# cule/multimot_track

Hardware: AMD Instinct MI355X
Metric: KITTI RGB-D frames/sec (ego+object poses) at 1/2/4/8 GPUs; CPU ref fps (higher is better)
Workload: dtype u8

## Files before the change

### multimot_track_amd/csrc/mmt_ba.hip

```cpp

#include <hip/hip_runtime.h>

#include <algorithm>
#include <cfloat>
#include <chrono>
#include <cstdio>
#include <climits>
#include <cmath>
#include <cstring>
#include <map>

#include "mmt_ba.h"
#include "mmt_devmath.h"
#include "mmt_internal.h"

namespace mmt {

namespace {

constexpr int kBAThreads = 512;
constexpr int kBAWaves = kBAThreads / 64;
constexpr int kLdsRows = 96;

struct BAWork {
// ... 126 lines not shown
  Jp[0][0] = x * y / z_2 * c.fx;
  Jp[0][1] = -(1 + (x * x / z_2)) * c.fx;
  Jp[0][2] = y / z * c.fx;
  Jp[0][3] = -1. / z * c.fx;
  Jp[0][4] = 0;
  Jp[0][5] = x / z_2 * c.fx;
  Jp[1][0] = (1 + y * y / z_2) * c.fy;
  Jp[1][1] = -x * y / z_2 * c.fy;
  Jp[1][2] = -x / z * c.fy;
  Jp[1][3] = 0;
  Jp[1][4] = -1. / z * c.fy;
  Jp[1][5] = y / z_2 * c.fy;
  if (stereo) {
    Jp[2][0] = Jp[0][0] - c.bf * y / z_2;
    Jp[2][1] = Jp[0][1] + c.bf * x / z_2;
    Jp[2][2] = Jp[0][2];
    Jp[2][3] = Jp[0][3];
    Jp[2][4] = 0;
    Jp[2][5] = Jp[0][5] - c.bf / z_2;
  } else {
#pragma unroll
    for (int k = 0; k < 6; k++) Jp[2][k] = 0;
  }
}

__device__ __forceinline__ void inverse3(const double (&m)[9], double (&r)[9]) {
#define COF(i, j)                                                                           \
  (m[3 * (((i) + 1) % 3) + ((j) + 1) % 3] * m[3 * (((i) + 2) % 3) + ((j) + 2) % 3] -         \
   m[3 * (((i) + 1) % 3) + ((j) + 2) % 3] * m[3 * (((i) + 2) % 3) + ((j) + 1) % 3])
  const double c0 = COF(0, 0), c1 = COF(1, 0), c2 = COF(2, 0);
  const double det = c0 * m[0] + c1 * m[3] + c2 * m[6];
  const double invdet = 1.0 / det;
  r[0] = c0 * invdet;
  r[1] = c1 * invdet;
  r[2] = c2 * invdet;
  r[3] = COF(0, 1) * invdet;
  r[4] = COF(1, 1) * invdet;
  r[5] = COF(2, 1) * invdet;
  r[6] = COF(0, 2) * invdet;
  r[7] = COF(1, 2) * invdet;
  r[8] = COF(2, 2) * invdet;
#undef COF
}

__device__ __forceinline__ double wg_sum1(double v, double* part) {
  v = wave_sum_dpp(v);
  const int lane = threadIdx.x & 63, wave = threadIdx.x >> 6;
  if (lane == 0) part[wave] = v;
  __syncthreads();
  double s = 0;
#pragma unroll
  for (int w = 0; w < kBAWaves; w++) s += part[w];
  __syncthreads();
  return s;
}

__device__ __forceinline__ double wg_max1(double v, double* part) {
#pragma unroll
  for (int o = 32; o > 0; o >>= 1) v = fmax(v, __shfl_xor(v, o, 64));
  const int lane = threadIdx.x & 63, wave = threadIdx.x >> 6;
  if (lane == 0) part[wave] = v;
  __syncthreads();
  double m = 0;
#pragma unroll
  for (int w = 0; w < kBAWaves; w++) m = fmax(m, part[w]);
  __syncthreads();
  return m;
}

__device__ __forceinline__ void wave_sync_lds() {
  __builtin_amdgcn_fence(__ATOMIC_RELEASE, "wavefront");
  __builtin_amdgcn_wave_barrier();
  __builtin_amdgcn_fence(__ATOMIC_ACQUIRE, "wavefront");
}

}

namespace {

constexpr int kMkThreads = 256;
constexpr int kMkWaves = kMkThreads / 64;
constexpr int kMkSolveThreads = 512;
constexpr int kMkDecideThreads = 1024;

struct BAState {
  int done, round, iter, qmax, need_lin, lam_init, cb, ok2, nBad, nact;
  int spec_ok;
  int it_done[2], trials[2];
  double lambda, ni, chk, currentChi, iniChi, scale_p;
  long long prof[8];
};

struct BAWork2 {
  BAState* st;
  DSE3* pose;
  double* X;
  double* Hll;
  double* bl;
  double* Dinv;
  double* err;
  double* Hpl;
  double* Hpe;
  double* Y;
  double* cv;
  double* Hpp;
  double* bp;
  double* cvs;
  double* Sblk;
  double* x;
  double* S;
  double* vec;
  const int4* kitem;
  const int* kitem_start;
  const int4* bitem;
  const int* bitem_start;
  int n_kitem, n_bitem;
  double* Hpart;
  double* Spart;
  double* cvpart;
  double* linpart;
  double* p4part;
  unsigned* p4cnt;
  uint8_t* level;
  int* eopt;
  uint8_t* kf_act;
  uint8_t* pt_act;
  int gP;
  int gPp;
  const int* heavy;
  int n_heavy;
  double* hres;
  int spec;
};

template <int K, int NW>
__device__ __forceinline__ void wg_sumK(const double (&v)[K], double* part, double* out) {
  const int lane = threadIdx.x & 63, wave = threadIdx.x >> 6;
  double mine = 0;
#pragma unroll
  for (int q = 0; q < K; q++) {
    const double s = wave_sum_dpp(v[q]);
    if (lane == q) mine = s;
  }
  if (lane < K) part[wave * K + lane] = mine;
  __syncthreads();
  if ((int)threadIdx.x < K) {
    double s = 0;
#pragma unroll
    for (int w = 0; w < NW; w++) s += part[w * K + threadIdx.x];
    out[threadIdx.x] = s;
  }
  __syncthreads();
}

template <int NW>
__device__ __forceinline__ double wg_maxN(double v, double* part) {
#pragma unroll
  for (int o = 32; o > 0; o >>= 1) v = fmax(v, __shfl_xor(v, o, 64));
  const int lane = threadIdx.x & 63, wave = threadIdx.x >> 6;
  if (lane == 0) part[wave] = v;
  __syncthreads();
  double m = 0;
#pragma unroll
  for (int w = 0; w < NW; w++) m = fmax(m, part[w]);
  __syncthreads();
  return m;
}

__device__ __forceinline__ int ba2_diag_q(int r) { return 6 * r - r * (r - 1) / 2; }

template <int U = 8>
__device__ __forceinline__ double ordered_sum(const double* base, size_t stride, int b, int e) {
  double s = 0;
  for (int it = b; it < e; it += U) {
    double v[U];
#pragma unroll
    for (int u = 0; u < U; u++) v[u] = base[stride * (size_t)min(it + u, e - 1)];
#pragma unroll
    for (int u = 0; u < U; u++)
      if (it + u < e) s += v[u];
  }
  return s;
}

__device__ __forceinline__ double ba2_hsum(const BAWork2& w, int a, int q) {
  return ordered_sum(w.Hpart + q, 27, w.kitem_start[a], w.kitem_start[a + 1]);
}

__device__ __forceinline__ double ba2_lambda_init(const BADesc& d, const BAWork2& w, double* sh) {
  if (threadIdx.x < 64) {
    double m = 0;
    for (int g = threadIdx.x; g < w.gP; g += 64) m = fmax(m, w.linpart[2 * g + 1]);
    for (int q = threadIdx.x; q < 6 * d.n_opt; q += 64) {
      const int a = q / 6;
      if (w.kf_act[d.opt_kf[a]]) m = fmax(m, fabs(ba2_hsum(w, a, ba2_diag_q(q % 6))));
    }
#pragma unroll
    for (int o = 32; o > 0; o >>= 1) m = fmax(m, __shfl_xor(m, o, 64));
    if (threadIdx.x == 0) *sh = 1e-5 * m;
  }
  __syncthreads();
  return *sh;
}

__device__ __forceinline__ Cam ba_cam(const BADesc& d) { return Cam{d.fx, d.fy, d.cx, d.cy, d.bf}; }

__device__ __forceinline__ double huber_mono() { return (double)(float)sqrt(5.991); }
__device__ __forceinline__ double huber_stereo() { return (double)(float)sqrt(7.815); }

__global__ __launch_bounds__(kMkThreads) void k_ba2_init(BADesc d, BAWork2 w) {
  const int gt = blockIdx.x * kMkThreads + threadIdx.x, gs = gridDim.x * kMkThreads;
  const size_t n6 = 6 * (size_t)d.n_opt;
  for (int j = gt; j < d.n_pt; j += gs) {
    for (int r = 0; r < 3; r++) {
// ... 113 lines not shown
  return r0;
}

template <int K>
__device__ __forceinline__ void ba2_wave_ordered_add(double* sh, int lane, int n, const bool valid,
                                                     const double (&v)[K], double (&sum)[K]) {
#pragma unroll
  for (int q = 0; q < K; q++) sh[K * lane + q] = valid ? v[q] : 0.0;
  const unsigned long long vb = __ballot(valid);
  __builtin_amdgcn_fence(__ATOMIC_RELEASE, "wavefront");
  __builtin_amdgcn_wave_barrier();
  __builtin_amdgcn_fence(__ATOMIC_ACQUIRE, "wavefront");
  for (int k = 0; k < n; k++) {
    if (!((vb >> k) & 1ull)) continue;
#pragma unroll
    for (int q = 0; q < K; q++) sum[q] += sh[K * k + q];
  }
  __builtin_amdgcn_fence(__ATOMIC_RELEASE, "wavefront");
  __builtin_amdgcn_wave_barrier();
}

__device__ __forceinline__ double ba2_lin_point(const BADesc& d, const BAWork2& w, int j,
                                               const DSE3* pose, const double (&X)[3], bool robust,
                                               int lb, double* mx) {
  double* Hpl_b = w.Hpl + (size_t)lb * 18 * d.n_edge;
  double* Hpe_b = w.Hpe + (size_t)lb * 27 * d.n_edge;
  double chi = 0;
  {
    double hl[9] = {0, 0, 0, 0, 0, 0, 0, 0, 0}, b3[3] = {0, 0, 0};
    for (int e = d.pt_start[j]; e < d.pt_start[j + 1]; e++) {
      if (w.level[e]) continue;
      double acc9[9], g3[3];
      chi += ba2_lin_edge(d, w, e, pose, X, robust, Hpl_b, Hpe_b, acc9, g3);
#pragma unroll
      for (int q = 0; q < 9; q++) hl[q] += acc9[q];
#pragma unroll
      for (int a = 0; a < 3; a++) b3[a] += g3[a];
    }
    double* Hll_b = w.Hll + (size_t)lb * 9 * d.n_pt;
    double* bl_b = w.bl + (size_t)lb * 3 * d.n_pt;
#pragma unroll
    for (int q = 0; q < 9; q++) Hll_b[9 * (size_t)j + q] = hl[q];
#pragma unroll
    for (int q = 0; q < 3; q++) bl_b[3 * (size_t)j + q] = b3[q];
    *mx = fmax(fabs(hl[0]), fmax(fabs(hl[4]), fabs(hl[8])));
  }
  return chi;
}

__device__ __forceinline__ double ba2_lin_point_wave(const BADesc& d, const BAWork2& w, int j,
                                                    const DSE3* pose, const double (&X)[3],
                                                    bool robust, int lb, double* mx, double* sh) {
  const int lane = threadIdx.x & 63;
  double* Hpl_b = w.Hpl + (size_t)lb * 18 * d.n_edge;
  double* Hpe_b = w.Hpe + (size_t)lb * 27 * d.n_edge;
  double sum[13] = {0, 0, 0, 0, 0, 0, 0, 0, 0, 0, 0, 0, 0};
  const int e1 = d.pt_start[j + 1];
  for (int e0 = d.pt_start[j]; e0 < e1; e0 += 64) {
    const int e = e0 + lane;
    const bool valid = e < e1 && !w.level[e];
    double v[13];
    if (valid) {
      double acc9[9], g3[3];
      v[0] = ba2_lin_edge(d, w, e, pose, X, robust, Hpl_b, Hpe_b, acc9, g3);
#pragma unroll
      for (int q = 0; q < 9; q++) v[1 + q] = acc9[q];
#pragma unroll
      for (int q = 0; q < 3; q++) v[10 + q] = g3[q];
    }
    ba2_wave_ordered_add<13>(sh, lane, min(64, e1 - e0), valid, v, sum);
  }
  if (lane == 0) {
    double* Hll_b = w.Hll + (size_t)lb * 9 * d.n_pt;
    double* bl_b = w.bl + (size_t)lb * 3 * d.n_pt;
#pragma unroll
    for (int q = 0; q < 9; q++) Hll_b[9 * (size_t)j + q] = sum[1 + q];
#pragma unroll
    for (int q = 0; q < 3; q++) bl_b[3 * (size_t)j + q] = sum[10 + q];
  }
  *mx = fmax(fabs(sum[1]), fmax(fabs(sum[5]), fabs(sum[9])));
  return sum[0];
}

__global__ __launch_bounds__(kMkThreads) void k_ba2_lin(BADesc d, BAWork2 w) {
  __shared__ double s_part[2 * kMkWaves];
  const BAState* st = w.st;
  if (st->done || !st->need_lin || st->spec_ok) return;
  const bool robust = st->round == 0;
  const int cb = st->cb;
  const DSE3* pose = w.pose + (size_t)cb * d.n_kf;
  const double* Xc = w.X + (size_t)cb * 3 * d.n_pt;
  const int j = blockIdx.x * kMkThreads + threadIdx.x;
  double chi = 0, mx = 0;
  if (j < d.n_pt) {
    double m = 0;
    if (ba2_heavy(d, j)) {
      chi = w.hres[2 * (size_t)j];
      m = w.hres[2 * (size_t)j + 1];
    } else {
      const double X[3] = {Xc[3 * (size_t)j], Xc[3 * (size_t)j + 1], Xc[3 * (size_t)j + 2]};
      chi = ba2_lin_point(d, w, j, pose, X, robust, cb, &m);
    }
    if (w.pt_act[j]) mx = m;
  }
  const double cs = wave_sum_dpp(chi);
  const int lane = threadIdx.x & 63, wave = threadIdx.x >> 6;
  if (lane == 0) s_part[wave] = cs;
  const double m = wg_maxN<kMkWaves>(mx, s_part + kMkWaves);
  if (threadIdx.x == 0) {
    double t = 0;
#pragma unroll
    for (int q = 0; q < kMkWaves; q++) t += s_part[q];
    w.linpart[2 * blockIdx.x] = t;
    w.linpart[2 * blockIdx.x + 1] = m;
  }
}

__global__ __launch_bounds__(kMkThreads) void k_ba2_lin_heavy(BADesc d, BAWork2 w) {
  __shared__ double s_stage[kMkWaves][64 * 13];
  const BAState* st = w.st;
  if (st->done || !st->need_lin || st->spec_ok) return;
  const int wave = threadIdx.x >> 6;
  const int hi = (int)blockIdx.x * kMkWaves + wave;
  if (hi >= w.n_heavy) return;
  const int cb = st->cb;
  const DSE3* pose = w.pose + (size_t)cb * d.n_kf;
  const double* Xc = w.X + (size_t)cb * 3 * d.n_pt;
  const int j = w.heavy[hi];
  const double X[3] = {Xc[3 * (size_t)j], Xc[3 * (size_t)j + 1], Xc[3 * (size_t)j + 2]};
  double m = 0;
  const double c = ba2_lin_point_wave(d, w, j, pose, X, st->round == 0, cb, &m, s_stage[wave]);
  if ((threadIdx.x & 63) == 0) {
    w.hres[2 * (size_t)j] = c;
    w.hres[2 * (size_t)j + 1] = m;
  }
}

__global__ __launch_bounds__(kMkThreads) void k_ba2_kfsum(BADesc d, BAWork2 w) {
  __shared__ double s_part[27 * kMkWaves];
  __shared__ double s_out[32];
  const BAState* st = w.st;
  if (st->done || !st->need_lin) return;
  const int4 it = w.kitem[blockIdx.x];
  const int t = it.y + threadIdx.x;
  double acc[27];
#pragma unroll
  for (int q = 0; q < 27; q++) acc[q] = 0;
  if (t < it.z) {
    const int e = d.kf_edges[t];
    if (!w.level[e]) {
      const double* h = &w.Hpe[(size_t)st->cb * 27 * d.n_edge + 27 * (size_t)e];
#pragma unroll
      for (int q = 0; q < 27; q++) acc[q] = h[q];
    }
  }
  wg_sumK<27, kMkWaves>(acc, s_part, s_out);
  if (threadIdx.x < 27) w.Hpart[27 * (size_t)blockIdx.x + threadIdx.x] = s_out[threadIdx.x];
}

__global__ __launch_bounds__(kMkThreads) void k_ba2_p1(BADesc d, BAWork2 w) {
  const BAState* st = w.st;
  if (st->done) return;
  __shared__ double s_lam;
  const double lambda = st->lam_init ? ba2_lambda_init(d, w, &s_lam) : st->lambda;
  const bool heavy_wg = (int)blockIdx.x >= w.gPp;
  const int lane = threadIdx.x & 63;
  int j = blockIdx.x * kMkThreads + threadIdx.x;
  if (heavy_wg) {
    const int hi = ((int)blockIdx.x - w.gPp) * kMkWaves + (int)(threadIdx.x >> 6);
    j = hi < w.n_heavy ? w.heavy[hi] : d.n_pt;
  } else if (j < d.n_pt && ba2_heavy(d, j)) {
    return;
  }
  if (j >= d.n_pt || !w.pt_act[j]) return;
  const int cb = st->cb;
  const double* Hll_c = w.Hll + (size_t)cb * 9 * d.n_pt;
  const double* bl_c = w.bl + (size_t)cb * 3 * d.n_pt;
  const double* Hpl_c = w.Hpl + (size_t)cb * 18 * d.n_edge;
  double Dm[9], Di[9];
#pragma unroll
  for (int q = 0; q < 9; q++) Dm[q] = Hll_c[9 * (size_t)j + q] + ((q % 4) == 0 ? lambda : 0.0);
  inverse3(Dm, Di);
  if (!heavy_wg || lane == 0) {
#pragma unroll
    for (int q = 0; q < 9; q++) w.Dinv[9 * (size_t)j + q] = Di[q];
  }
  const double* b3 = &bl_c[3 * (size_t)j];
  double db[3];
#pragma unroll
  for (int a = 0; a < 3; a++) db[a] = Di[3 * a] * b3[0] + Di[3 * a + 1] * b3[1] + Di[3 * a + 2] * b3[2];
  const int eb = d.pt_start[j] + (heavy_wg ? lane : 0), es = heavy_wg ? 64 : 1;
  for (int e = eb; e < d.pt_start[j + 1]; e += es) {
    if (w.level[e] || w.eopt[e] < 0) continue;
    const double* B = &Hpl_c[18 * (size_t)e];
    double* Ye = &w.Y[18 * (size_t)e];
    double* ce = &w.cv[6 * (size_t)e];
#pragma unroll
    for (int r = 0; r < 6; r++) {
      const double b0 = B[3 * r], b1 = B[3 * r + 1], b2 = B[3 * r + 2];
#pragma unroll
      for (int c = 0; c < 3; c++) Ye[3 * r + c] = b0 * Di[c] + b1 * Di[3 + c] + b2 * Di[6 + c];
      ce[r] = b0 * db[0] + b1 * db[1] + b2 * db[2];
    }
  }
}

__global__ __launch_bounds__(kMkThreads) void k_ba2_p2(BADesc d, BAWork2 w) {
  __shared__ double s_part[36 * kMkWaves];
  __shared__ double s_out[64];
  const BAState* st = w.st;
  if (st->done) return;
  if ((int)blockIdx.x < w.n_bitem) {
    const int4 it = w.bitem[blockIdx.x];
    const int t = it.y + threadIdx.x;
    double acc[36];
#pragma unroll
    for (int q = 0; q < 36; q++) acc[q] = 0;
    if (t < it.z) {
      const int2 tr = d.trip[t];
      if (!w.level[tr.x] && !w.level[tr.y]) {
        const double* Ye = &w.Y[18 * (size_t)tr.x];
        const double* B2 = &w.Hpl[(size_t)st->cb * 18 * d.n_edge + 18 * (size_t)tr.y];
        double h2[18], y[18];
#pragma unroll
        for (int q = 0; q < 18; q++) {
          h2[q] = B2[q];
          y[q] = Ye[q];
        }
#pragma unroll
        for (int r = 0; r < 6; r++)
#pragma unroll
          for (int c = 0; c < 6; c++)
            acc[6 * r + c] = y[3 * r] * h2[3 * c] + y[3 * r + 1] * h2[3 * c + 1] + y[3 * r + 2] * h2[3 * c + 2];
      }
    }
    wg_sumK<36, kMkWaves>(acc, s_part, s_out);
    if (threadIdx.x < 36) w.Spart[36 * (size_t)blockIdx.x + threadIdx.x] = s_out[threadIdx.x];
  } else {
    const int ki = blockIdx.x - w.n_bitem;
    const int4 it = w.kitem[ki];
    const int t = it.y + threadIdx.x;
    double cs[6] = {0, 0, 0, 0, 0, 0};
    if (t < it.z) {
      const int e = d.kf_edges[t];
      if (!w.level[e]) {
#pragma unroll
        for (int r = 0; r < 6; r++) cs[r] = w.cv[6 * (size_t)e + r];
      }
    }
    wg_sumK<6, kMkWaves>(cs, s_part, s_out);
    if (threadIdx.x < 6) w.cvpart[6 * (size_t)ki + threadIdx.x] = s_out[threadIdx.x];
  }
// ... 381 lines not shown
  const double* bl_c = w.bl + (size_t)cb * 3 * d.n_pt;
  const double* Hpl_c = w.Hpl + (size_t)cb * 18 * d.n_edge;
  const int lane = threadIdx.x & 63;
  double chi = 0, sc = 0;
  double X[3] = {Xc[3 * (size_t)j], Xc[3 * (size_t)j + 1], Xc[3 * (size_t)j + 2]};
  if (w.pt_act[j]) {
    double* xl = &w.x[n6 + 3 * (size_t)j];
    const double bl3[3] = {bl_c[3 * (size_t)j], bl_c[3 * (size_t)j + 1], bl_c[3 * (size_t)j + 2]};
    double xv3[3];
    if (ok2) {
      double Di[9];
#pragma unroll
      for (int q = 0; q < 9; q++) Di[q] = w.Dinv[9 * (size_t)j + q];
      double cl[3] = {bl3[0], bl3[1], bl3[2]};
      auto add_edge = [&](int e, int a) {
        double B[18];
#pragma unroll
        for (int q = 0; q < 18; q++) B[q] = Hpl_c[18 * (size_t)e + q];
#pragma unroll
        for (int c = 0; c < 3; c++)
#pragma unroll
          for (int r = 0; r < 6; r++) cl[c] += B[3 * r + c] * (-w.x[6 * a + r]);
      };
      if (!WAVE) {
        for (int e = d.pt_start[j]; e < d.pt_start[j + 1]; e++) {
          const int a = w.eopt[e];
          if (w.level[e] || a < 0) continue;
          add_edge(e, a);
        }
      } else {
        const int e1 = d.pt_start[j + 1];
        for (int e0 = d.pt_start[j]; e0 < e1; e0 += 64) {
          const int e = e0 + lane;
          const bool take = e < e1 && !w.level[e] && w.eopt[e] >= 0;
          unsigned long long m = __ballot(take);
          while (m) {
            const int k = __builtin_ctzll(m);
            m &= m - 1;
            add_edge(e0 + k, w.eopt[e0 + k]);
          }
        }
      }
#pragma unroll
      for (int a = 0; a < 3; a++)
        xv3[a] = Di[3 * a] * cl[0] + Di[3 * a + 1] * cl[1] + Di[3 * a + 2] * cl[2];
      if (!WAVE || lane == 0) {
#pragma unroll
        for (int a = 0; a < 3; a++) xl[a] = xv3[a];
      }
    } else {
#pragma unroll
      for (int a = 0; a < 3; a++) xv3[a] = xl[a];
    }
#pragma unroll
    for (int r = 0; r < 3; r++) {
      const double xv = xv3[r];
      sc += xv * (lambda * xv + bl3[r]);
      X[r] += xv;
    }
    if (!WAVE) {
      for (int e = d.pt_start[j]; e < d.pt_start[j + 1]; e++)
        if (!w.level[e]) chi += ba2_trial_edge(d, w, e, tri, X, robust);
    } else {
      double sum[1] = {0};
      const int e1 = d.pt_start[j + 1];
      for (int e0 = d.pt_start[j]; e0 < e1; e0 += 64) {
        const int e = e0 + lane;
        const bool valid = e < e1 && !w.level[e];
        double v[1] = {0};
        if (valid) v[0] = ba2_trial_edge(d, w, e, tri, X, robust);
        ba2_wave_ordered_add<1>(sh, lane, min(64, e1 - e0), valid, v, sum);
      }
      chi = sum[0];
    }
  }
  if (!WAVE || lane == 0) {
#pragma unroll
    for (int r = 0; r < 3; r++) Xt[3 * (size_t)j + r] = X[r];
  }
  *chi_out = chi;
  *sc_out = sc;
}

__global__ __launch_bounds__(kMkThreads) void k_ba2_p4_heavy(BADesc d, BAWork2 w) {
  __shared__ double s_stage[kMkWaves][64];
  if (w.st->done) return;
  const int wave = threadIdx.x >> 6;
  const int hi = (int)blockIdx.x * kMkWaves + wave;
  if (hi >= w.n_heavy) return;
  const int j = w.heavy[hi];
  double chi, sc;
  ba2_trial_point<true>(d, w, j, s_stage[wave], &chi, &sc);
  if ((threadIdx.x & 63) == 0) {
    w.hres[2 * (size_t)j] = chi;
    w.hres[2 * (size_t)j + 1] = sc;
  }
}

__global__ __launch_bounds__(kMkThreads) void k_ba2_p4(BADesc d, BAWork2 w) {
  __shared__ double s_part[2 * kMkWaves];
  __shared__ int s_last;
  const BAState* st = w.st;
  if (st->done) return;
  const int lane = threadIdx.x & 63, wave = threadIdx.x >> 6;
  const int j = blockIdx.x * kMkThreads + threadIdx.x;
  double chi = 0, sc = 0;
  if (j < d.n_pt) {
    if (ba2_heavy(d, j)) {
      chi = w.hres[2 * (size_t)j];
      sc = w.hres[2 * (size_t)j + 1];
    } else {
      ba2_trial_point<false>(d, w, j, nullptr, &chi, &sc);
    }
  }
  const double a = wave_sum_dpp(chi), b = wave_sum_dpp(sc);
  if (lane == 0) {
    s_part[2 * wave] = a;
    s_part[2 * wave + 1] = b;
  }
  __threadfence();
  __syncthreads();
  if (threadIdx.x == 0) {
    double t0 = 0, t1 = 0;
#pragma unroll
    for (int q = 0; q < kMkWaves; q++) {
      t0 += s_part[2 * q];
      t1 += s_part[2 * q + 1];
    }
    w.p4part[2 * blockIdx.x] = t0;
    w.p4part[2 * blockIdx.x + 1] = t1;
    __threadfence();
    const unsigned done = atomicAdd(w.p4cnt, 1u);
    s_last = done == (unsigned)gridDim.x - 1;
    if (s_last) __threadfence();
  }
  __syncthreads();
  if (!s_last) return;
  ba2_decide<kMkThreads>(d, w);
  if (threadIdx.x == 0) *w.p4cnt = 0;
}

__global__ __launch_bounds__(kMkDecideThreads) void k_ba2_finish(BADesc d, BAWork2 w) {
  __shared__ double s_part[kMkDecideThreads / 64];
  const int tid = threadIdx.x;
  const int cb = w.st->cb;
  const DSE3* pose = w.pose + (size_t)cb * d.n_kf;
  const double* Xc = w.X + (size_t)cb * 3 * d.n_pt;
  int nerase = 0;
  for (int e = tid; e < d.n_edge; e += kMkDecideThreads) {
    const bool stereo = !(d.e_obs[3 * (size_t)e + 2] < 0);
    const double chi = edge_chi2(&w.err[3 * (size_t)e], (double)d.e_s[e], stereo);
    double pc[3];
    se3_map(pose[d.e_kf[e]], &Xc[3 * (size_t)d.e_pt[e]], pc);
    const bool er = chi > (stereo ? 7.815 : 5.991) || !(pc[2] > 0.0);
    d.erase[e] = er ? 1 : 0;
    nerase += er;
  }
  for (int k = tid; k < d.n_kf; k += kMkDecideThreads) dse3_to_float(pose[k], d.T_out + 16 * (size_t)k);
  for (int q = tid; q < 3 * d.n_pt; q += kMkDecideThreads) d.X_out[q] = (float)Xc[q];
  const double na = wave_sum_dpp((double)nerase);
  if ((tid & 63) == 0) s_part[tid >> 6] = na;
  __syncthreads();
  if (tid == 0) {
    double t = 0;
    for (int q = 0; q < kMkDecideThreads / 64; q++) t += s_part[q];
    const BAState& s = *w.st;
    d.stats[0] = s.it_done[0];
    d.stats[1] = s.it_done[1];
    d.stats[2] = s.trials[0];
    d.stats[3] = s.trials[1];
    d.stats[4] = (int)t;
  }
}

}

size_t ba_workspace_bytes(int n_kf, int n_pt, int n_edge, int n_opt) {
  const size_t n6 = 6 * (size_t)n_opt;
  const size_t nd = 14 * (size_t)n_kf + (3 + 3 + 9 + 3 + 9) * (size_t)n_pt +
                    (3 + 18 + 18 + 6) * (size_t)n_edge + 42 * (size_t)n_opt + n6 + 3 * (size_t)n_pt +
                    n6 * n6 + 3 * n6;
  return 8 * nd + (size_t)n_edge + n_kf + n_pt + 64;
}

size_t ba2_workspace_bytes(int n_kf, int n_pt, int n_edge, int n_opt, int n_blk, int gP) {
  auto a = [](size_t x) { return (x + 15) & ~(size_t)15; };
  const size_t n6 = 6 * (size_t)n_opt;
  return a(sizeof(BAState)) + a(sizeof(DSE3) * 2 * (size_t)n_kf) + a(8 * 6 * (size_t)n_pt) +
         a(8 * 18 * (size_t)n_pt) + a(8 * 6 * (size_t)n_pt) + a(8 * 9 * (size_t)n_pt) +
         a(8 * 3 * (size_t)n_edge) + a(8 * 36 * (size_t)n_edge) + a(8 * 54 * (size_t)n_edge) +
         a(8 * 18 * (size_t)n_edge) + a(8 * 6 * (size_t)n_edge) + a(8 * 36 * (size_t)n_opt) +
         a(8 * 6 * (size_t)n_opt) + a(8 * 6 * (size_t)n_opt) + a(8 * 36 * (size_t)n_blk) +
         a(8 * (n6 + 3 * (size_t)n_pt)) + a(8 * n6 * n6) + a(8 * 7 * n6) + 2 * a(8 * 2 * (size_t)gP) +
         a((size_t)n_edge) + a(4 * (size_t)n_edge) + a((size_t)n_kf) + a((size_t)n_pt) + a(16) + 64;
}


static size_t al16(size_t x) { return (x + 15) & ~(size_t)15; }

BARunner::~BARunner() {
  if (d_ws2_) (void)hipFree(d_ws2_);
  if (h_flag_) (void)hipHostFree(h_flag_);
  if (d_up_) (void)hipFree(d_up_);
  if (d_dn_) (void)hipFree(d_dn_);
  if (d_ws_) (void)hipFree(d_ws_);
  if (h_up_) (void)hipHostFree(h_up_);
  if (h_dn_) (void)hipHostFree(h_dn_);
}

void BARunner::grow(uint8_t*& d, uint8_t*& h, size_t& cap, size_t need, hipStream_t st) {
  if (need <= cap && d) return;
  MMT_HIP(hipStreamSynchronize(st));
  if (d) (void)hipFree(d);
  if (h) (void)hipHostFree(h);
  cap = std::max(need + (need >> 1), (size_t)1 << 16);
  MMT_HIP(hipMalloc((void**)&d, cap));
  MMT_HIP(hipHostMalloc((void**)&h, cap, hipHostMallocDefault));
}

namespace {
double ba_now_us() {
// ... 65 lines not shown
      for (size_t p2 = p1; p2 < col.size(); p2++)
        trip[bfill[bid[(size_t)col[p1].first * nO + col[p2].first]]++] =
            make_int2(col[p1].second, col[p2].second);
    }
  }
  std::vector<int4> kitem, bitem;
  std::vector<int> kitem_start{0}, bitem_start{0};
  for (int a = 0; a < nO; a++) {
    for (int t = kf_start[a]; t < kf_start[a + 1]; t += 256)
      kitem.push_back(make_int4(a, t, std::min(t + 256, kf_start[a + 1]), 0));
    kitem_start.push_back((int)kitem.size());
  }
  for (size_t bk = 0; bk + 1 < blk_start.size(); bk++) {
    for (int t = blk_start[bk]; t < blk_start[bk + 1]; t += 256)
      bitem.push_back(make_int4((int)bk, t, std::min(t + 256, blk_start[bk + 1]), 0));
    bitem_start.push_back((int)bitem.size());
  }
  std::vector<int> heavy;
  for (int j = 0; j < nP; j++)
    if (pt_start[j + 1] - pt_start[j] > kBaHeavy) heavy.push_back(j);
  struct Seg {
    size_t bytes;
    const void* src;
  };
  const Seg segs[] = {{64 * (size_t)nK, P.Tcw},           {4 * opt_of.size(), opt_of.data()},
                      {4 * opt_kf.size(), opt_kf.data()}, {12 * (size_t)nP, P.Xw},
                      {4 * pt_start.size(), pt_start.data()}, {4 * (size_t)nE, P.e_pt},
                      {4 * (size_t)nE, P.e_kf},           {12 * (size_t)nE, P.e_obs},
                      {4 * (size_t)nE, P.e_s},            {4 * kf_start.size(), kf_start.data()},
                      {4 * kf_edges.size(), kf_edges.data()}, {4 * blk_ab.size(), blk_ab.data()},
                      {4 * blk_start.size(), blk_start.data()}, {8 * trip.size(), trip.data()},
                      {16 * kitem.size(), kitem.data()}, {4 * kitem_start.size(), kitem_start.data()},
                      {16 * bitem.size(), bitem.data()}, {4 * bitem_start.size(), bitem_start.data()},
                      {4 * heavy.size(), heavy.data()}};
  constexpr int nseg = sizeof(segs) / sizeof(segs[0]);
  size_t off[nseg], tot = 0;
  for (int i = 0; i < nseg; i++) {
    off[i] = tot;
    tot += al16(segs[i].bytes);
  }
  grow(d_up_, h_up_, up_cap_, tot, st);
  for (int i = 0; i < nseg; i++)
    if (segs[i].bytes) memcpy(h_up_ + off[i], segs[i].src, segs[i].bytes);
  const size_t o_X = al16(64 * (size_t)nK), o_er = o_X + al16(12 * (size_t)nP),
               o_st = o_er + al16((size_t)nE), dn = o_st + 64;
  grow(d_dn_, h_dn_, dn_cap_, dn, st);
  const size_t wsb = ba_workspace_bytes(nK, nP, nE, nO);
  if (wsb > ws_cap_ || !d_ws_) {
    MMT_HIP(hipStreamSynchronize(st));
    if (d_ws_) (void)hipFree(d_ws_);
    ws_cap_ = wsb + (wsb >> 1);
    MMT_HIP(hipMalloc((void**)&d_ws_, ws_cap_));
  }
  MMT_HIP(hipMemcpyAsync(d_up_, h_up_, tot, hipMemcpyHostToDevice, st));
  BADesc d;
  memset(&d, 0, sizeof(d));
  d.n_kf = nK;
  d.n_pt = nP;
  d.n_edge = nE;
  d.n_opt = nO;
  d.n_blk = nblocks;
  const uint8_t* u = d_up_;
  d.Tcw = (const float*)(u + off[0]);
  d.opt_of = (const int*)(u + off[1]);
  d.opt_kf = (const int*)(u + off[2]);
  d.Xw = (const float*)(u + off[3]);
  d.pt_start = (const int*)(u + off[4]);
  d.e_pt = (const int*)(u + off[5]);
  d.e_kf = (const int*)(u + off[6]);
  d.e_obs = (const float*)(u + off[7]);
  d.e_s = (const float*)(u + off[8]);
  d.kf_start = (const int*)(u + off[9]);
  d.kf_edges = (const int*)(u + off[10]);
  d.blk_ab = (const int*)(u + off[11]);
  d.blk_start = (const int*)(u + off[12]);
  d.trip = (const int2*)(u + off[13]);
  d.fx = P.fx; d.fy = P.fy; d.cx = P.cx; d.cy = P.cy; d.bf = P.bf;
  d.ws = d_ws_;
  d.T_out = (float*)d_dn_;
  d.X_out = (float*)(d_dn_ + o_X);
  d.erase = d_dn_ + o_er;
  d.stats = (int*)(d_dn_ + o_st);
  {
    const int gPp = std::max(1, (nP + kMkThreads - 1) / kMkThreads);
    const int gH = ((int)heavy.size() + kMkWaves - 1) / kMkWaves;
    const int gP = gPp;
    const int n6 = 6 * nO, nblk = nblocks;
    const size_t wsb2 = ba2_workspace_bytes(nK, nP, nE, nO, nblk, gP) +
                        8 * (27 + 6) * kitem.size() + 8 * 36 * bitem.size() + 16 * (size_t)nP +
                        64 * 4;
    if (wsb2 > ws2_cap_ || !d_ws2_) {
      MMT_HIP(hipStreamSynchronize(st));
      if (d_ws2_) (void)hipFree(d_ws2_);
      ws2_cap_ = wsb2 + (wsb2 >> 1);
      MMT_HIP(hipMalloc((void**)&d_ws2_, ws2_cap_));
    }
    if (!h_flag_) MMT_HIP(hipHostMalloc((void**)&h_flag_, 64, hipHostMallocDefault));
    BAWork2 w;
    uint8_t* p = d_ws2_;
    auto take = [&](size_t bytes) {
      uint8_t* r = p;
      p += al16(bytes);
      return r;
    };
    w.st = (BAState*)take(sizeof(BAState));
    w.pose = (DSE3*)take(sizeof(DSE3) * 2 * (size_t)nK);
    w.X = (double*)take(8 * 6 * (size_t)nP);
    w.Hll = (double*)take(8 * 2 * 9 * (size_t)nP);
    w.bl = (double*)take(8 * 2 * 3 * (size_t)nP);
    w.Dinv = (double*)take(8 * 9 * (size_t)nP);
    w.err = (double*)take(8 * 3 * (size_t)nE);
    w.Hpl = (double*)take(8 * 2 * 18 * (size_t)nE);
    w.Hpe = (double*)take(8 * 2 * 27 * (size_t)nE);
    w.Y = (double*)take(8 * 18 * (size_t)nE);
    w.cv = (double*)take(8 * 6 * (size_t)nE);
    w.Hpp = (double*)take(8 * 36 * (size_t)nO);
    w.bp = (double*)take(8 * 6 * (size_t)nO);
    w.cvs = (double*)take(8 * 6 * (size_t)nO);
    w.Sblk = (double*)take(8 * 36 * (size_t)nblk);
    w.kitem = (const int4*)(u + off[14]);
    w.kitem_start = (const int*)(u + off[15]);
    w.bitem = (const int4*)(u + off[16]);
    w.bitem_start = (const int*)(u + off[17]);
    w.n_kitem = (int)kitem.size();
    w.n_bitem = (int)bitem.size();
    w.Hpart = (double*)take(8 * 27 * kitem.size());
    w.Spart = (double*)take(8 * 36 * bitem.size());
    w.cvpart = (double*)take(8 * 6 * kitem.size());
    w.x = (double*)take(8 * ((size_t)n6 + 3 * (size_t)nP));
    w.S = (double*)take(8 * (size_t)n6 * n6);
    w.vec = (double*)take(8 * 7 * (size_t)n6);
    w.linpart = (double*)take(8 * 2 * (size_t)gP);
    w.p4part = (double*)take(8 * 2 * (size_t)gP);
    w.p4cnt = (unsigned*)take(16);
    w.level = take((size_t)nE);
    w.eopt = (int*)take(4 * (size_t)nE);
    w.kf_act = take((size_t)nK);
    w.pt_act = take((size_t)nP);
    w.gP = gP;
    w.gPp = gPp;
    w.heavy = (const int*)(u + off[18]);
    w.n_heavy = (int)heavy.size();
    w.hres = (double*)take(16 * (size_t)nP);
    w.spec = 0;
    const double tp1 = hp.on ? ba_now_us() : 0;
    double t_launch = 0, t_wait = 0;
    hipLaunchKernelGGL(k_ba2_init, dim3(gPp), dim3(kMkThreads), 0, st, d, w);
    MMT_HIP(hipGetLastError());
    int slots = 0;
    for (bool done = nE == 0; !done;) {
      const int batch = slots == 0 ? 15 : 4;
      const double tl = hp.on ? ba_now_us() : 0;
      for (int b = 0; b < batch; b++) {
        if (gH > 0) hipLaunchKernelGGL(k_ba2_lin_heavy, dim3(gH), dim3(kMkThreads), 0, st, d, w);
        hipLaunchKernelGGL(k_ba2_lin, dim3(gPp), dim3(kMkThreads), 0, st, d, w);
        if (w.n_kitem > 0)
          hipLaunchKernelGGL(k_ba2_kfsum, dim3(w.n_kitem), dim3(kMkThreads), 0, st, d, w);
        hipLaunchKernelGGL(k_ba2_p1, dim3(gPp + gH), dim3(kMkThreads), 0, st, d, w);
        if (w.n_bitem + w.n_kitem > 0)
          hipLaunchKernelGGL(k_ba2_p2, dim3(w.n_bitem + w.n_kitem), dim3(kMkThreads), 0, st, d, w);
        hipLaunchKernelGGL(k_ba2_p3, dim3(1), dim3(kMkSolveThreads), 0, st, d, w);
        if (gH > 0) hipLaunchKernelGGL(k_ba2_p4_heavy, dim3(gH), dim3(kMkThreads), 0, st, d, w);
        hipLaunchKernelGGL(k_ba2_p4, dim3(gPp), dim3(kMkThreads), 0, st, d, w);
      }
      MMT_HIP(hipGetLastError());
      slots += batch;
      MMT_HIP(hipMemcpyAsync(h_flag_, &w.st->done, sizeof(int), hipMemcpyDeviceToHost, st));
      const double tw = hp.on ? ba_now_us() : 0;
      MMT_HIP(hipStreamSynchronize(st));
      if (hp.on) {
        t_launch += tw - tl;
        t_wait += ba_now_us() - tw;
      }
      done = *h_flag_ != 0;
      if (!done && slots >= 160) throw DeviceError("local BA: the LM did not finish in 150 trials");
    }
    hipLaunchKernelGGL(k_ba2_finish, dim3(1), dim3(kMkDecideThreads), 0, st, d, w);
    MMT_HIP(hipGetLastError());
    if (hp.on) {
      hp.t[0] += tp1 - tp0;
      hp.t[1] += t_launch;
      hp.t[2] += t_wait;
      hp.slots += slots;
      BAState hs;
      MMT_HIP(hipMemcpy(&hs, w.st, sizeof(hs), hipMemcpyDeviceToHost));
      for (int q = 0; q < 5; q++) hp.p3[q] += hs.prof[q];
    }
  }
  MMT_HIP(hipMemcpyAsync(h_dn_, d_dn_, dn, hipMemcpyDeviceToHost, st));
  MMT_HIP(hipStreamSynchronize(st));
  memcpy(T_out, h_dn_, 64 * (size_t)nK);
  memcpy(X_out, h_dn_ + o_X, 12 * (size_t)nP);
  memcpy(erase, h_dn_ + o_er, (size_t)nE);
  memcpy(stats, h_dn_ + o_st, 5 * sizeof(int));
  if (hp.on) {
    hp.t[4] += ba_now_us() - tp0;
    if (++hp.n % 32 == 0)
      fprintf(stderr, "[mmt ba profile] %ld solves, host us per solve: layout + upload %.1f, "
              "launches %.1f, waits %.1f, total %.1f; %.1f trial slots per solve\n", hp.n,
              hp.t[0] / hp.n, hp.t[1] / hp.n, hp.t[2] / hp.n, hp.t[4] / hp.n,
              (double)hp.slots / hp.n);
    if (hp.on && hp.n % 32 == 0)
      fprintf(stderr, "[mmt ba profile] k_ba2_p3 us per solve: partials %.1f, assembly %.1f, "
              "LDL^T %.1f, substitutions %.1f, poses + state %.1f\n", hp.p3[0] * 0.01 / hp.n,
              hp.p3[1] * 0.01 / hp.n, hp.p3[2] * 0.01 / hp.n, hp.p3[3] * 0.01 / hp.n,
              hp.p3[4] * 0.01 / hp.n);
  }
}

}
```

Measured before the change: 688.6.

## Merge heavy-point kernels into light ones and defer partial reductions

Folds the separate heavy-point linearize and trial kernels into the main per-point kernels: extra workgroups handle heavy points wave-wise, and all per-point results go to a shared pres buffer. The chi/max reduction of linearization moves into extra blocks of the kfsum kernel. In p4, the last-arriving block now computes the per-block partial sums itself before deciding, using explicit agent-scope fences. This cuts two kernel launches per LM iteration, at the cost of a serial partial-sum pass in the last block and an added dependency through global memory.

```diff
diff --git a/multimot_track_amd/csrc/mmt_ba.hip b/multimot_track_amd/csrc/mmt_ba.hip
--- a/multimot_track_amd/csrc/mmt_ba.hip
+++ b/multimot_track_amd/csrc/mmt_ba.hip
@@ -232,6 +232,12 @@
 constexpr int kMkWaves = kMkThreads / 64;
 constexpr int kMkSolveThreads = 512;
 constexpr int kMkDecideThreads = 1024;
+#ifndef MMT_BA_PT_THREADS
+#define MMT_BA_PT_THREADS 256
+#endif
+constexpr int kPtThreads = MMT_BA_PT_THREADS;
+constexpr int kPtWaves = kPtThreads / 64;
+static_assert(kPtThreads % 64 == 0 && kPtThreads >= 64 && kPtThreads <= 1024, "whole waves");
 
 struct BAState {
   int done, round, iter, qmax, need_lin, lam_init, cb, ok2, nBad, nact;
@@ -279,7 +285,7 @@
   int gPp;
   const int* heavy;
   int n_heavy;
-  double* hres;
+  double* pres;
   int spec;
 };
 
@@ -559,57 +565,31 @@
   return sum[0];
 }
 
-__global__ __launch_bounds__(kMkThreads) void k_ba2_lin(BADesc d, BAWork2 w) {
-  __shared__ double s_part[2 * kMkWaves];
+__global__ __launch_bounds__(kPtThreads) void k_ba2_lin(BADesc d, BAWork2 w) {
+  __shared__ double s_stage[kPtWaves][64 * 13];
   const BAState* st = w.st;
   if (st->done || !st->need_lin || st->spec_ok) return;
   const bool robust = st->round == 0;
   const int cb = st->cb;
   const DSE3* pose = w.pose + (size_t)cb * d.n_kf;
   const double* Xc = w.X + (size_t)cb * 3 * d.n_pt;
-  const int j = blockIdx.x * kMkThreads + threadIdx.x;
-  double chi = 0, mx = 0;
-  if (j < d.n_pt) {
-    double m = 0;
-    if (ba2_heavy(d, j)) {
-      chi = w.hres[2 * (size_t)j];
-      m = w.hres[2 * (size_t)j + 1];
-    } else {
-      const double X[3] = {Xc[3 * (size_t)j], Xc[3 * (size_t)j + 1], Xc[3 * (size_t)j + 2]};
-      chi = ba2_lin_point(d, w, j, pose, X, robust, cb, &m);
-    }
-    if (w.pt_act[j]) mx = m;
-  }
-  const double cs = wave_sum_dpp(chi);
-  const int lane = threadIdx.x & 63, wave = threadIdx.x >> 6;
-  if (lane == 0) s_part[wave] = cs;
-  const double m = wg_maxN<kMkWaves>(mx, s_part + kMkWaves);
-  if (threadIdx.x == 0) {
-    double t = 0;
-#pragma unroll
-    for (int q = 0; q < kMkWaves; q++) t += s_part[q];
-    w.linpart[2 * blockIdx.x] = t;
-    w.linpart[2 * blockIdx.x + 1] = m;
-  }
-}
-
-__global__ __launch_bounds__(kMkThreads) void k_ba2_lin_heavy(BADesc d, BAWork2 w) {
-  __shared__ double s_stage[kMkWaves][64 * 13];
-  const BAState* st = w.st;
-  if (st->done || !st->need_lin || st->spec_ok) return;
+  const bool heavy_wg = (int)blockIdx.x >= w.gPp;
   const int wave = threadIdx.x >> 6;
-  const int hi = (int)blockIdx.x * kMkWaves + wave;
-  if (hi >= w.n_heavy) return;
-  const int cb = st->cb;
-  const DSE3* pose = w.pose + (size_t)cb * d.n_kf;
-  const double* Xc = w.X + (size_t)cb * 3 * d.n_pt;
-  const int j = w.heavy[hi];
+  int j = blockIdx.x * kPtThreads + threadIdx.x;
+  if (heavy_wg) {
+    const int hi = ((int)blockIdx.x - w.gPp) * kPtWaves + wave;
+    if (hi >= w.n_heavy) return;
+    j = w.heavy[hi];
+  } else if (j >= d.n_pt || ba2_heavy(d, j)) {
+    return;
+  }
   const double X[3] = {Xc[3 * (size_t)j], Xc[3 * (size_t)j + 1], Xc[3 * (size_t)j + 2]};
   double m = 0;
-  const double c = ba2_lin_point_wave(d, w, j, pose, X, st->round == 0, cb, &m, s_stage[wave]);
-  if ((threadIdx.x & 63) == 0) {
-    w.hres[2 * (size_t)j] = c;
-    w.hres[2 * (size_t)j + 1] = m;
+  const double c = heavy_wg ? ba2_lin_point_wave(d, w, j, pose, X, robust, cb, &m, s_stage[wave])
+                            : ba2_lin_point(d, w, j, pose, X, robust, cb, &m);
+  if (!heavy_wg || (threadIdx.x & 63) == 0) {
+    w.pres[2 * (size_t)j] = c;
+    w.pres[2 * (size_t)j + 1] = m;
   }
 }
 
@@ -618,6 +598,28 @@
   __shared__ double s_out[32];
   const BAState* st = w.st;
   if (st->done || !st->need_lin) return;
+  if ((int)blockIdx.x >= w.n_kitem) {
+    if (st->spec_ok) return;
+    const int g = (int)blockIdx.x - w.n_kitem;
+    const int j = g * kMkThreads + threadIdx.x;
+    double chi = 0, mx = 0;
+    if (j < d.n_pt) {
+      chi = w.pres[2 * (size_t)j];
+      if (w.pt_act[j]) mx = w.pres[2 * (size_t)j + 1];
+    }
+    const double cs = wave_sum_dpp(chi);
+    const int lane = threadIdx.x & 63, wave = threadIdx.x >> 6;
+    if (lane == 0) s_part[wave] = cs;
+    const double m = wg_maxN<kMkWaves>(mx, s_part + kMkWaves);
+    if (threadIdx.x == 0) {
+      double t = 0;
+#pragma unroll
+      for (int q = 0; q < kMkWaves; q++) t += s_part[q];
+      w.linpart[2 * g] = t;
+      w.linpart[2 * g + 1] = m;
+    }
+    return;
+  }
   const int4 it = w.kitem[blockIdx.x];
   const int t = it.y + threadIdx.x;
   double acc[27];
@@ -635,16 +637,16 @@
   if (threadIdx.x < 27) w.Hpart[27 * (size_t)blockIdx.x + threadIdx.x] = s_out[threadIdx.x];
 }
 
-__global__ __launch_bounds__(kMkThreads) void k_ba2_p1(BADesc d, BAWork2 w) {
+__global__ __launch_bounds__(kPtThreads) void k_ba2_p1(BADesc d, BAWork2 w) {
   const BAState* st = w.st;
   if (st->done) return;
   __shared__ double s_lam;
   const double lambda = st->lam_init ? ba2_lambda_init(d, w, &s_lam) : st->lambda;
   const bool heavy_wg = (int)blockIdx.x >= w.gPp;
   const int lane = threadIdx.x & 63;
-  int j = blockIdx.x * kMkThreads + threadIdx.x;
+  int j = blockIdx.x * kPtThreads + threadIdx.x;
   if (heavy_wg) {
-    const int hi = ((int)blockIdx.x - w.gPp) * kMkWaves + (int)(threadIdx.x >> 6);
+    const int hi = ((int)blockIdx.x - w.gPp) * kPtWaves + (int)(threadIdx.x >> 6);
     j = hi < w.n_heavy ? w.heavy[hi] : d.n_pt;
   } else if (j < d.n_pt && ba2_heavy(d, j)) {
     return;
@@ -1192,61 +1194,81 @@
   *sc_out = sc;
 }
 
-__global__ __launch_bounds__(kMkThreads) void k_ba2_p4_heavy(BADesc d, BAWork2 w) {
-  __shared__ double s_stage[kMkWaves][64];
-  if (w.st->done) return;
-  const int wave = threadIdx.x >> 6;
-  const int hi = (int)blockIdx.x * kMkWaves + wave;
-  if (hi >= w.n_heavy) return;
-  const int j = w.heavy[hi];
-  double chi, sc;
-  ba2_trial_point<true>(d, w, j, s_stage[wave], &chi, &sc);
-  if ((threadIdx.x & 63) == 0) {
-    w.hres[2 * (size_t)j] = chi;
-    w.hres[2 * (size_t)j + 1] = sc;
-  }
-}
-
-__global__ __launch_bounds__(kMkThreads) void k_ba2_p4(BADesc d, BAWork2 w) {
-  __shared__ double s_part[2 * kMkWaves];
+template <int NT>
+__device__ __forceinline__ void ba2_p4_partials(const BADesc& d, const BAWork2& w) {
+  constexpr int NW = NT / 64, U = 4;
+  const int lane = threadIdx.x & 63, wave = threadIdx.x >> 6;
+  const double2* pres2 = reinterpret_cast<const double2*>(w.pres);
+  for (int g0 = wave * U; g0 < w.gP; g0 += NW * U) {
+    double2 v[U][kMkWaves];
+#pragma unroll
+    for (int u = 0; u < U; u++)
+#pragma unroll
+      for (int q = 0; q < kMkWaves; q++) {
+        const int j = (g0 + u) * kMkThreads + 64 * q + lane;
+        v[u][q] = pres2[min(j, d.n_pt - 1)];
+      }
+#pragma unroll
+    for (int u = 0; u < U; u++) {
+      double t0 = 0, t1 = 0;
+#pragma unroll
+      for (int q = 0; q < kMkWaves; q++) {
+        const bool in = (g0 + u) * kMkThreads + 64 * q + lane < d.n_pt;
+        t0 += wave_sum_dpp(in ? v[u][q].x : 0.0);
+        t1 += wave_sum_dpp(in ? v[u][q].y : 0.0);
+      }
+      if (lane == 0 && g0 + u < w.gP) {
+        w.p4part[2 * (g0 + u)] = t0;
+        w.p4part[2 * (g0 + u) + 1] = t1;
+      }
+    }
+  }
+}
+
+__global__ __launch_bounds__(kPtThreads) void k_ba2_p4(BADesc d, BAWork2 w) {
+  __shared__ double s_stage[kPtWaves][64];
   __shared__ int s_last;
   const BAState* st = w.st;
   if (st->done) return;
   const int lane = threadIdx.x & 63, wave = threadIdx.x >> 6;
-  const int j = blockIdx.x * kMkThreads + threadIdx.x;
-  double chi = 0, sc = 0;
-  if (j < d.n_pt) {
-    if (ba2_heavy(d, j)) {
-      chi = w.hres[2 * (size_t)j];
-      sc = w.hres[2 * (size_t)j + 1];
-    } else {
+  const bool heavy_wg = (int)blockIdx.x >= w.gPp;
+  int j = blockIdx.x * kPtThreads + threadIdx.x;
+  bool mine = j < d.n_pt && !ba2_heavy(d, j);
+  if (heavy_wg) {
+    const int hi = ((int)blockIdx.x - w.gPp) * kPtWaves + wave;
+    mine = hi < w.n_heavy;
+    if (mine) j = w.heavy[hi];
+  }
+  if (mine) {
+    double chi, sc;
+    if (heavy_wg)
+      ba2_trial_point<true>(d, w, j, s_stage[wave], &chi, &sc);
+    else
       ba2_trial_point<false>(d, w, j, nullptr, &chi, &sc);
-    }
-  }
-  const double a = wave_sum_dpp(chi), b = wave_sum_dpp(sc);
-  if (lane == 0) {
-    s_part[2 * wave] = a;
-    s_part[2 * wave + 1] = b;
-  }
-  __threadfence();
+    if (!heavy_wg || lane == 0) {
+      w.pres[2 * (size_t)j] = chi;
+      w.pres[2 * (size_t)j + 1] = sc;
+    }
+  }
+  asm volatile("s_waitcnt vmcnt(0)" ::: "memory");
   __syncthreads();
   if (threadIdx.x == 0) {
-    double t0 = 0, t1 = 0;
-#pragma unroll
-    for (int q = 0; q < kMkWaves; q++) {
-      t0 += s_part[2 * q];
-      t1 += s_part[2 * q + 1];
-    }
-    w.p4part[2 * blockIdx.x] = t0;
-    w.p4part[2 * blockIdx.x + 1] = t1;
-    __threadfence();
-    const unsigned done = atomicAdd(w.p4cnt, 1u);
-    s_last = done == (unsigned)gridDim.x - 1;
-    if (s_last) __threadfence();
+    __builtin_amdgcn_fence(__ATOMIC_RELEASE, "agent");
+    asm volatile("s_waitcnt vmcnt(0)" ::: "memory");
+    const unsigned done =
+        __hip_atomic_fetch_add(w.p4cnt, 1u, __ATOMIC_RELAXED, __HIP_MEMORY_SCOPE_AGENT);
+    const int last = done == (unsigned)gridDim.x - 1;
+    if (last) {
+      __builtin_amdgcn_fence(__ATOMIC_ACQUIRE, "agent");
+      asm volatile("s_waitcnt vmcnt(0)" ::: "memory");
+    }
+    s_last = last;
   }
   __syncthreads();
   if (!s_last) return;
-  ba2_decide<kMkThreads>(d, w);
+  ba2_p4_partials<kPtThreads>(d, w);
+  __syncthreads();
+  ba2_decide<kPtThreads>(d, w);
   if (threadIdx.x == 0) *w.p4cnt = 0;
 }
 
@@ -1478,9 +1500,9 @@
   d.erase = d_dn_ + o_er;
   d.stats = (int*)(d_dn_ + o_st);
   {
-    const int gPp = std::max(1, (nP + kMkThreads - 1) / kMkThreads);
-    const int gH = ((int)heavy.size() + kMkWaves - 1) / kMkWaves;
-    const int gP = gPp;
+    const int gPp = std::max(1, (nP + kPtThreads - 1) / kPtThreads);
+    const int gH = ((int)heavy.size() + kPtWaves - 1) / kPtWaves;
+    const int gP = std::max(1, (nP + kMkThreads - 1) / kMkThreads);
     const int n6 = 6 * nO, nblk = nblocks;
     const size_t wsb2 = ba2_workspace_bytes(nK, nP, nE, nO, nblk, gP) +
                         8 * (27 + 6) * kitem.size() + 8 * 36 * bitem.size() + 16 * (size_t)nP +
@@ -1537,7 +1559,7 @@
     w.gPp = gPp;
     w.heavy = (const int*)(u + off[18]);
     w.n_heavy = (int)heavy.size();
-    w.hres = (double*)take(16 * (size_t)nP);
+    w.pres = (double*)take(16 * (size_t)nP);
     w.spec = 0;
     const double tp1 = hp.on ? ba_now_us() : 0;
     double t_launch = 0, t_wait = 0;
@@ -1548,16 +1570,13 @@
       const int batch = slots == 0 ? 15 : 4;
       const double tl = hp.on ? ba_now_us() : 0;
       for (int b = 0; b < batch; b++) {
-        if (gH > 0) hipLaunchKernelGGL(k_ba2_lin_heavy, dim3(gH), dim3(kMkThreads), 0, st, d, w);
-        hipLaunchKernelGGL(k_ba2_lin, dim3(gPp), dim3(kMkThreads), 0, st, d, w);
-        if (w.n_kitem > 0)
-          hipLaunchKernelGGL(k_ba2_kfsum, dim3(w.n_kitem), dim3(kMkThreads), 0, st, d, w);
-        hipLaunchKernelGGL(k_ba2_p1, dim3(gPp + gH), dim3(kMkThreads), 0, st, d, w);
+        hipLaunchKernelGGL(k_ba2_lin, dim3(gPp + gH), dim3(kPtThreads), 0, st, d, w);
+        hipLaunchKernelGGL(k_ba2_kfsum, dim3(w.n_kitem + gP), dim3(kMkThreads), 0, st, d, w);
+        hipLaunchKernelGGL(k_ba2_p1, dim3(gPp + gH), dim3(kPtThreads), 0, st, d, w);
         if (w.n_bitem + w.n_kitem > 0)
           hipLaunchKernelGGL(k_ba2_p2, dim3(w.n_bitem + w.n_kitem), dim3(kMkThreads), 0, st, d, w);
         hipLaunchKernelGGL(k_ba2_p3, dim3(1), dim3(kMkSolveThreads), 0, st, d, w);
-        if (gH > 0) hipLaunchKernelGGL(k_ba2_p4_heavy, dim3(gH), dim3(kMkThreads), 0, st, d, w);
-        hipLaunchKernelGGL(k_ba2_p4, dim3(gPp), dim3(kMkThreads), 0, st, d, w);
+        hipLaunchKernelGGL(k_ba2_p4, dim3(gPp + gH), dim3(kPtThreads), 0, st, d, w);
       }
       MMT_HIP(hipGetLastError());
       slots += batch;
```

Result: faster. 711.2 (median of 6 runs) (+3.3%).
